# Ulixes-8/UNet-Implementations

Hardware: AMD Instinct MI355X
Metric: images/sec (512x512, bs/GPU=8) Our_UNet train step (higher is better)
Workload: dtype f32; 1 GPU; Our_UNet 6-stage 3-class 512x512 bs=8/GPU fp32 train step (fwd + Dice/wCE loss + bwd + SGD-Nesterov), train mode, HIP conv/IN/upsample kernels; global_batch=8, parallelism=dp1, world=1

## Files before the change

include/unet_hip.h:

```cpp
#ifndef UNET_HIP_H_
#define UNET_HIP_H_

#include <stddef.h>
#include <stdint.h>

#ifdef __cplusplus
extern "C" {
#endif

#define UNET_ABI_VERSION 11

#define UNET_OK 0
#define UNET_E_INVALID (-1)
#define UNET_E_LAUNCH (-2)
#define UNET_E_WORKSPACE (-3)

typedef void* unet_stream_t;

const char* unet_last_error(void);
int unet_abi_version(void);
int unet_device_count(void);

int unet_debug_set_chunk_limit(int64_t bytes);

// ... 235 lines not shown
                                const uint16_t* dy, float* dw_oihw, void* workspace,
                                size_t workspace_bytes, int N, int H, int W, int Cout,
                                unet_stream_t stream);

size_t unet_stem_in_bwd_weight_fold_workspace_bytes(int N, int H, int W, int Cout);
int unet_stem_in_bwd_weight_fold(const float* x, const uint8_t* image_hwc, const float* mean3,
                                 const float* std3, const float* g, const float* y,
                                 const float* mean, const float* rstd, const float* gamma,
                                 const float* beta, const float* mask, float slope,
                                 const void* partial, int tiles, float* dw_oihw, float* dgamma,
                                 float* dbeta, float* dbias, void* workspace,
                                 size_t workspace_bytes, int N, int H, int W, int Cout,
                                 unet_stream_t stream);

int unet_conv_in_bwd_weight_fold32_supported(int N, int H, int W, int Cx, int Cout);
size_t unet_conv_in_bwd_weight_fold32_workspace_bytes(int N, int H, int W);
int unet_conv_in_bwd_weight_fold32(const unet_act_src* x, float slope_x, float* g, const float* y,
                                   const float* mean, const float* rstd, const float* gamma,
                                   const float* beta, const float* mask, float slope,
                                   const void* partial, int tiles, float* dw_oihw, int ci_offset,
                                   int Cin_total, float* dgamma, float* dbeta, float* dbias,
                                   void* workspace, size_t workspace_bytes, int N, int H, int W,
                                   unet_stream_t stream);

int unet_conv_in_bwd_weight(const unet_act_src* x, float slope, const float* dy, float* dw_oihw,
                            int ci_offset, int Cin_total, int ksize, int stride, void* workspace,
                            size_t workspace_bytes, int N, int H, int W, int Cout,
                            unet_stream_t stream);
int unet_conv_in_bwd_weight_bf16x3(const unet_act_src* x, float slope, const float* dy, float* dw_oihw,
                            int ci_offset, int Cin_total, int ksize, int stride, void* workspace,
                            size_t workspace_bytes, int N, int H, int W, int Cout,
                            unet_stream_t stream);

int unet_upsample2x_in_fwd(const unet_act_src* x, float slope, float* up, int N, int h, int w,
                           unet_stream_t stream);

int unet_upsample2x_bwd_taps(const float* dy, float* D, int N, int h, int w, int C,
                             unet_stream_t stream);
int unet_resize_bilinear_fwd(const float* x, float* y, int planes, int h, int w, int H, int W,
                             unet_stream_t stream);
int unet_resize_bilinear_bwd(const float* gy, float* gx, int planes, int h, int w, int H, int W,
                             unet_stream_t stream);
size_t unet_conv3x3_up_bwd_weight_workspace_bytes(int N, int h, int w, int Cx, int Cout);
int unet_conv3x3_up_bwd_weight(const unet_act_src* x, float slope, const float* D, float* dw_oihw,
                               int ci_offset, int Cin_total, void* workspace,
                               size_t workspace_bytes, int N, int h, int w, int Cout,
// ... 220 lines not shown
```

unet-implementations_amd/_lib.py:

```python
import ctypes
import os
import subprocess

_HERE = os.path.dirname(os.path.abspath(__file__))
LIB_PATH = os.environ.get("UNET_HIP_LIB") or os.path.join(_HERE, "libunet_hip.so")
CSRC = os.path.join(_HERE, "csrc")

ABI_VERSION = 11

_c = ctypes
_p = _c.c_void_p
_i = _c.c_int
_f = _c.c_float
_sz = _c.c_size_t
_i64 = _c.c_int64



class ActSrc(ctypes.Structure):
    _fields_ = [("x", _p), ("C", _i), ("alpha", _p), ("beta", _p)]


_ps = _c.POINTER(ActSrc)

# ... 130 lines not shown
                                     _i, _p]),
    "unet_conv3x3_up_bwd_data_b16": (_i, [_p, _p, _i, _i, _p, _i, _i, _i, _i, _i, _i, _p]),
    "unet_conv3x3_up_bwd_data_bs_b16": (_i, [_p, _p, _i, _i, _p, _i, _i, _i, _i, _i, _i, _pbs, _p]),
    "unet_conv3x3_up_bwd_data_bs_b16_wb": (_i, [_p, _p, _p, _i, _i, _p, _i, _i, _i, _i, _i, _i, _pbs,
                                           _p]),
    "unet_head1x1_in_fwd_b16": (_i, [_ps, _f, _p, _p, _p, _i, _i, _i, _p]),
    "unet_head1x1_in_bwd_b16": (_i, [_ps, _f, _p, _p, _p, _p, _p, _p, _sz, _i, _i, _i, _p]),
    "unet_upsample2x_bwd_taps": (_i, [_p, _p, _i, _i, _i, _i, _p]),
    "unet_conv3x3_up_bwd_weight_workspace_bytes": (_sz, [_i, _i, _i, _i, _i]),
    "unet_conv3x3_up_bwd_weight": (_i, [_ps, _f, _p, _p, _i, _i, _p, _sz, _i, _i, _i, _i, _p]),
    "unet_conv3x3_up_bwd_data": (_i, [_p, _p, _i, _i, _p, _i, _i, _i, _i, _i, _i, _p]),
    "unet_head1x1_in_fwd": (_i, [_ps, _f, _p, _p, _p, _i, _i, _i, _p]),
    "unet_head1x1_in_bwd": (_i, [_ps, _f, _p, _p, _p, _p, _p, _p, _sz, _i, _i, _i, _p]),
    "unet_head1x1_in_bwd_bs": (_i, [_ps, _f, _p, _p, _p, _p, _p, _p, _sz, _i, _i, _i, _pbs, _p]),
    "unet_head1x1_in_bwd_bs_b16": (_i, [_ps, _f, _p, _p, _p, _p, _p, _p, _sz, _i, _i, _i, _pbs, _p]),
    "unet_stem_in_bwd_weight_fold_workspace_bytes": (_sz, [_i, _i, _i, _i]),
    "unet_stem_in_bwd_weight_fold": (_i, [_p, _p, _c.POINTER(_f), _c.POINTER(_f), _p, _p, _p, _p, _p,
                                          _p, _p, _f, _p, _i, _p, _p, _p, _p, _p, _sz, _i, _i, _i,
                                          _i, _p]),
    "unet_conv_in_bwd_weight_fold32_supported": (_i, [_i, _i, _i, _i, _i]),
    "unet_conv_in_bwd_weight_fold32_workspace_bytes": (_sz, [_i, _i, _i]),
    "unet_conv_in_bwd_weight_fold32": (_i, [_ps, _f, _p, _p, _p, _p, _p, _p, _p, _f, _p, _i, _p, _i,
                                            _i, _p, _p, _p, _p, _sz, _i, _i, _i, _p]),
    "unet_instnorm_bwd_merge_partials": (_i, [_p, _i, _p, _p, _i, _i, _i, _p]),
    "unet_head1x1_in_bwd_fold_workspace_bytes": (_sz, [_i, _i, _i]),
    "unet_head1x1_in_bwd_fold": (_i, [_ps, _f, _p, _p, _p, _p, _p, _p, _p, _p, _p, _sz, _i, _i, _i,
                                      _pbs, _p]),
    "unet_recon3x3_fwd": (_i, [_ps, _i, _f, _p, _p, _p, _i, _i, _i, _i, _p]),
    "unet_recon3x3_bwd_workspace_bytes": (_sz, [_i, _i, _i]),
    "unet_recon3x3_bwd": (_i, [_ps, _i, _f, _p, _p, _p, _p, _p, _p, _p, _sz, _i, _i, _i, _i, _pbs,
                               _p]),
    "unet_mse_loss_workspace_bytes": (_sz, [_i, _i, _i, _i]),
    "unet_mse_loss_fwd": (_i, [_p, _p, _i, _p, _p, _p, _sz, _i, _i, _i, _i, _p]),
    "unet_mse_loss_grad": (_i, [_p, _p, _i, _p, _p, _i, _i, _i, _i, _p]),
    "unet_adam_step": (_i, [_p, _p, _p, _p, _i64, _p, _i, _p]),
    "unet_ssim_workspace_bytes": (_sz, [_i, _i, _i, _i]),
    "unet_ssim_fwd": (_i, [_p, _p, _i, _c.POINTER(_f), _f, _f, _p, _p, _p, _c.c_double,
                           _c.c_double, _p, _sz, _i, _i, _i, _i, _p]),
    "unet_ssim_grad": (_i, [_p, _p, _i, _c.POINTER(_f), _f, _f, _p, _i, _c.c_double, _c.c_double,
                            _p, _i, _i, _i, _i, _p]),
    "unet_perceptual_prep": (_i, [_p, _p, _i, _c.POINTER(_f), _c.POINTER(_f), _p, _i, _i, _i, _p]),
    "unet_relu_maxpool2x2_fwd": (_i, [_p, _p, _i, _i, _i, _i, _p]),
    "unet_feature_mse_workspace_bytes": (_sz, [_i, _i, _i, _i]),
    "unet_feature_mse_fwd": (_i, [_p, _p, _p, _sz, _i, _i, _i, _i, _p]),
    "unet_perceptual_relu_bwd": (_i, [_p, _p, _f, _p, _p, _p, _i, _i, _i, _i, _p]),
    "unet_perceptual_stem_bwd_data": (_i, [_p, _p, _c.POINTER(_f), _p, _i, _i, _i, _i, _p]),
# ... 54 lines not shown
```

unet-implementations_amd/csrc/conv_wgrad.hip:

```cpp
#include "conv_params.h"
#include <vector>
#include "lds_asm.h"
#include <type_traits>
#include <utility>

namespace {
using unet_conv::act4;
using unet_conv::act4f;
template <int I> using template_ic = std::integral_constant<int, I>;
template <int B, int... I, typename F>
__device__ __forceinline__ void for_range_impl(std::integer_sequence<int, I...>, F&& f) {
  (f(template_ic<B + I>{}), ...);
}
template <int B, int E, typename F>
__device__ __forceinline__ void for_range(F&& f) {
  for_range_impl<B>(std::make_integer_sequence<int, (E > B ? E - B : 0)>{}, f);
}

struct WgradParams {
  const float* x;
  const float* dy;
  float* partial;
  int Cx, Cout;
  int N, H, W, Ho, Wo;
// ... 1500 lines not shown
  static_assert(lds <= 160 * 1024, "stages exceed the CU's LDS");
  return with_bool(p.alpha != nullptr, [&](auto act) {
    return launch_kernel<
        conv_wgrad_kernel<CI_T, CO_T, S, STRIDE, decltype(act)::value, float, float, 8>>(
        "conv_wgrad(8 waves)", wgrad_grid(p), 512, lds, stream, p);
  });
}

template <int CI_T, int CO_T, int STRIDE>
int launch_wgrad8_s(const WgradParams& p, int S, hipStream_t stream) {
  constexpr int NSB = (CI_T / 32) * (CO_T / 32);
  constexpr int SMAX = NSB == 1 ? (STRIDE == 1 ? 128 : 32) : NSB == 2 ? 64 : (STRIDE == 1 ? 64 : 32);
  if constexpr (SMAX >= 128) if (S == 128) return launch_wgrad8<CI_T, CO_T, 128, STRIDE>(p, stream);
  if constexpr (SMAX >= 64) if (S == 64) return launch_wgrad8<CI_T, CO_T, 64, STRIDE>(p, stream);
  if (S == 32) return launch_wgrad8<CI_T, CO_T, 32, STRIDE>(p, stream);
  if (S == 16) return launch_wgrad8<CI_T, CO_T, 16, STRIDE>(p, stream);
  unet_set_error("conv_wgrad(8 waves): no instantiation for S=%d", S);
  return UNET_E_INVALID;
}

constexpr int WW_XP = 4 * 18, WW_DP = 2 * 16;
constexpr int WW_BUF = 16 * 512;
constexpr size_t WW_LDS = (size_t)(4 * WW_BUF + (WW_XP + WW_DP) * 64) * sizeof(float);

template <bool ACT>
__global__ __launch_bounds__(512, 2) void conv_wgrad_wino_kernel(const WgradParams p) {
  extern __shared__ __attribute__((aligned(16))) float smem[];
  float* Vs = smem;
  float* Es = smem + 2 * WW_BUF;
  float* Rx = smem + 4 * WW_BUF;
  float* Rd = Rx + WW_XP * 64;

  const int tid = threadIdx.x, lane = tid & 63, wave = tid >> 6;
  int bid = blockIdx.x;
  const int co_t = bid % p.co_tiles; bid /= p.co_tiles;
  const int ci_t = bid % p.ci_tiles; bid /= p.ci_tiles;
  const int sp = bid;
  const int ci0 = ci_t * 64, co0 = co_t * 64;
  const int g_begin = sp * p.segs_per_block;
  const int g_end = min(g_begin + p.segs_per_block, p.total_segs);
  const int cw = p.W >> 4, th = p.H >> 1;

  const int xshift = (p.W + 1) * p.Cx;
  const __amdgpu_buffer_rsrc_t rsx = __builtin_amdgcn_make_buffer_rsrc(
      const_cast<float*>(p.x) - xshift, 0, (int)(p.x_bytes + 4u * (unsigned)xshift), 0x00020000);
  const __amdgpu_buffer_rsrc_t rsd = __builtin_amdgcn_make_buffer_rsrc(
      const_cast<float*>(p.dy), 0, (int)p.dy_bytes, 0x00020000);

  const int grp4 = (tid & 15) * 4;
  unsigned voffx[3], fx[3];
  float* xdst[3];
#pragma unroll
  for (int i = 0; i < 3; ++i) {
    const int pix = (tid + 512 * i) >> 4;
    const int prow = pix / 18, pcol = pix - prow * 18;
    voffx[i] = (unsigned)((prow * p.W + pcol) * p.Cx + ci0 + grp4) * 4u;
    fx[i] = (prow == 0 ? 1u : 0u) | (prow == 3 ? 2u : 0u) | (pcol == 0 ? 4u : 0u) |
            (pcol == 17 ? 8u : 0u) | (pix >= WW_XP ? 16u : 0u);
    xdst[i] = Rx + (pix < WW_XP ? pix : 0) * 64 + grp4;
  }
  const bool slot2 = tid + 1024 < WW_XP * 16;
  const int d_pixl = tid >> 4;
  const unsigned voffd = (unsigned)(((d_pixl >> 4) * p.W + (d_pixl & 15)) * p.Cout + co0 + grp4) * 4u;
  float* const ddst = Rd + d_pixl * 64 + grp4;
  f32x4 rx[3], rd;
  float okf[3] = {1.f, 1.f, 1.f};
  f32x4 ca = {1.f, 1.f, 1.f, 1.f}, cb = {0.f, 0.f, 0.f, 0.f};
  int l_cc, l_tr, l_n, l_g = g_begin;
  {
    const int r = g_begin / cw;
    l_cc = g_begin - r * cw;
    l_n = r / th;
    l_tr = r - l_n * th;
  }
  auto load_raw = [&]() {
    const unsigned m = (l_tr == 0 ? 1u : 0u) | (l_tr == th - 1 ? 2u : 0u) | (l_cc == 0 ? 4u : 0u) |
                       (l_cc == cw - 1 ? 8u : 0u) | 16u;
    const int pixbase = (l_n * p.H + 2 * l_tr) * p.W + 16 * l_cc;
#pragma unroll
    for (int i = 0; i < 3; ++i) {
      const bool ok = (fx[i] & m) == 0u;
      okf[i] = ok ? 1.f : 0.f;
      rx[i] = __builtin_bit_cast(f32x4, __builtin_amdgcn_raw_buffer_load_b128(
                                            rsx, ok ? voffx[i] : 0x80000000u, pixbase * p.Cx * 4, 0));
    }
    rd = __builtin_bit_cast(f32x4, __builtin_amdgcn_raw_buffer_load_b128(rsd, voffd,
                                                                          pixbase * p.Cout * 4, 0));
    if (ACT) {
      const size_t o = (size_t)l_n * p.Cx + ci0;
      ca = *reinterpret_cast<const f32x4*>(p.alpha + o + grp4);
      cb = *reinterpret_cast<const f32x4*>(p.beta + o + grp4);
    }
    if (l_g + 1 < g_end) {
      ++l_g;
      if (++l_cc == cw) { l_cc = 0; if (++l_tr == th) { l_tr = 0; ++l_n; } }
    }
  };
  auto store_x = [&](auto ic) {
    constexpr int i = decltype(ic)::value;
    f32x4 v = rx[i];
    if (ACT) v = act4f(v, ca, cb, p.slope, okf[i]);
    if (i < 2 || slot2) *reinterpret_cast<f32x4*>(xdst[i]) = v;
  };
  auto store_d = [&]() { *reinterpret_cast<f32x4*>(ddst) = rd; };

  const int t_pair = wave & 3;
  const int t_half = __builtin_amdgcn_readfirstlane(wave >> 2);
  const unsigned t_xa = lds_addr(Rx + (4 * t_pair) * 64 + lane);
  const unsigned t_da = lds_addr(Rd + (4 * t_pair) * 64 + lane);
  const int t_off = t_pair * 128 + ((lane * 2) ^ (32 * (t_pair & 1)));
  float* const t_vdst = Vs + t_off;
  float* const t_edst = Es + t_off;
  f32x2v tq[6];
  auto tv_rd = [&](auto ac) {
    constexpr int a = decltype(ac)::value;
    constexpr int r0 = a == 0 ? 0 : (a == 1 ? 1 : (a == 2 ? 2 : 3));
    constexpr int r1 = a == 0 ? 2 : (a == 1 ? 2 : 1);
    tq[0] = lds_rd2st64<r0 * 18 + 0, r1 * 18 + 0>(t_xa);
    tq[1] = lds_rd2st64<r0 * 18 + 1, r1 * 18 + 1>(t_xa);
    tq[2] = lds_rd2st64<r0 * 18 + 2, r1 * 18 + 2>(t_xa);
    tq[3] = lds_rd2st64<r0 * 18 + 3, r1 * 18 + 3>(t_xa);
    tq[4] = lds_rd2st64<r0 * 18 + 4, r1 * 18 + 4>(t_xa);
    tq[5] = lds_rd2st64<r0 * 18 + 5, r1 * 18 + 5>(t_xa);
  };
  auto tv_wr = [&](auto ac, auto bc) {
    constexpr int a = decltype(ac)::value;
    constexpr int B = decltype(bc)::value;
// ... 86 lines not shown
      constexpr int NR = T ? n_reads(T ? x - 8 : 0, HF) : 0;
      if constexpr (x == 8) {
        asm volatile("s_waitcnt lgkmcnt(0)" ::: "memory");
        __builtin_amdgcn_s_barrier();
        asm volatile("" ::: "memory");
      }
      if constexpr (T) t_reads(template_ic<(T ? x - 8 : 0)>{}, hc);
      if constexpr (x + 1 < 16) frag(bc, template_ic<x + 1>{});
      lds_wait<(x + 1 < 16 ? 3 : 0) + NR>(fa[x & 1], fb0[x & 1], fb1[x & 1]);
      __builtin_amdgcn_sched_barrier(0);
      mm(xc);
      if constexpr (T) {
        lds_wait6<3>(tq[0], tq[1], tq[2], tq[3], tq[4], tq[5]);
        t_writes(template_ic<(T ? x - 8 : 0)>{}, hc, NB{});
      }
      if constexpr (x < 3) store_x(template_ic<(x < 3 ? x : 0)>{});
      if constexpr (x == 3) store_d();
      if constexpr (x == 4) load_raw();
      __builtin_amdgcn_sched_barrier(0);
    });
  };
  auto k_loop = [&](auto hc) {
    load_raw();
    for_range<0, 3>(store_x);
    store_d();
    load_raw();
    __syncthreads();
    for_range<0, 4>([&](auto kc) {
      t_reads(kc, hc);
      lds_wait6<0>(tq[0], tq[1], tq[2], tq[3], tq[4], tq[5]);
      t_writes(kc, hc, template_ic<0>{});
    });
    for (int g = g_begin; g < g_end; g += 2) {
      chunk_body(template_ic<0>{}, hc);
      if (g + 1 < g_end) chunk_body(template_ic<1>{}, hc);
    }
  };
  if (g_begin < g_end) {
    if (t_half == 0) k_loop(template_ic<0>{}); else k_loop(template_ic<1>{});
  }

#pragma unroll
  for (int x = 0; x < 16; ++x) {
    const float sc = (((x >> 2) == 1 || (x >> 2) == 2) ? 0.5f : 1.f) * (((x & 3) == 1 || (x & 3) == 2) ? 0.5f : 1.f);
    if (sc != 1.f) {
#pragma unroll
      for (int b = 0; b < 2; ++b) acc[x][b] *= sc;
    }
  }
#pragma unroll
  for (int b = 0; b < 2; ++b)
#pragma unroll
    for (int r = 0; r < 4; ++r) {
      float s[3][4];
#pragma unroll
      for (int j = 0; j < 4; ++j) {
        s[0][j] = acc[0 + j][b][r] + acc[4 + j][b][r] + acc[8 + j][b][r];
        s[1][j] = acc[4 + j][b][r] - acc[8 + j][b][r];
        s[2][j] = acc[4 + j][b][r] + acc[8 + j][b][r] + acc[12 + j][b][r];
      }
// ... 316 lines not shown
    return false;
  return c32 == 2 || (long long)N * (H / 8) * (W / 32) >= 256;
}
WgradPlan make_plan_wino32(int N, int H, int W) {
  WgradPlan pl{};
  const long long t = (long long)N * (H / 8) * (W / 32);
  pl.nw = 8; pl.ci_t = pl.co_t = 32; pl.npp = 1; pl.S = 16;
  pl.split = (int)(t < 256 ? t : 256);
  pl.total_segs = (int)t; pl.segs_per_block = 1; pl.segs_per_row = W / 32;
  pl.ws_floats = slab_ws_floats(pl.split, (size_t)9 * 32 * 32);
  return pl;
}
int launch_wgrad_wino32(const WgradParams& p, hipStream_t stream) {
  const int ntiles = p.N * (p.H / 8) * (p.W / 32);
  return with_bool(p.alpha != nullptr, [&](auto act) {
    return launch_kernel<conv_wgrad_wino32_kernel<decltype(act)::value>>(
        "conv_wgrad_wino32", dim3((unsigned)(ntiles < 256 ? ntiles : 256)), 512, WQ_LDS, stream, p,
        ntiles);
  });
}

int launch_wgrad_wino(const WgradParams& p, hipStream_t stream) {
  return with_bool(p.alpha != nullptr, [&](auto act) {
    return launch_kernel<conv_wgrad_wino_kernel<decltype(act)::value>>(
        "conv_wgrad_wino", wgrad_grid(p), 512, WW_LDS, stream, p);
  });
}

bool wgrad_wino_ok(int N, int H, int W, int Cx, int Cout, int stride) {
  if (stride != 1 || Cx % 64 || Cout % 64 || H % 2 || W % 16) return false;
  const long long chunks = (long long)N * (H / 2) * (W / 16);
  return chunks >= 32 && chunks < (1LL << 30);
}

WgradPlan make_plan_wino(int N, int H, int W, int Cx, int Cout) {
  WgradPlan pl{};
  pl.nw = 8; pl.ci_t = pl.co_t = 64; pl.npp = 2; pl.S = 16;
  pl.segs_per_row = W / 16;
  pl.total_segs = N * (H / 2) * (W / 16);
  pl.segs_per_block = ceil_div(
      pl.total_segs, wgrad_split(256, (Cx / 64) * (Cout / 64), ceil_div(pl.total_segs, 8)));
  return with_slabs(pl, Cx, Cout);
}

template <int CI_T, int CO_T, int S, int STRIDE>
int launch_wgrad(const WgradParams& p, hipStream_t stream) {
  constexpr int PW = (S - 1) * STRIDE + 3;
  constexpr size_t stages = 2 * (size_t)(3 * PW * CI_T + S * CO_T) * sizeof(float);
// ... 158 lines not shown
  }
  if (pl.ci_t == 32 && pl.co_t == 64) {
    if (stride == 1)
      return pl.S == 32 ? launch_wgrad<32, 64, 32, 1>(p, stream)
                        : launch_wgrad<32, 64, 16, 1>(p, stream);
    return pl.S == 32 ? launch_wgrad<32, 64, 32, 2>(p, stream)
                      : launch_wgrad<32, 64, 16, 2>(p, stream);
  }
  if (stride == 1)
    return pl.S == 32 ? launch_wgrad<64, 64, 32, 1>(p, stream)
                      : launch_wgrad<64, 64, 16, 1>(p, stream);
  return launch_wgrad<64, 64, 16, 2>(p, stream);
}

enum WgradForm { WF_STEM, WF_WINO, WF_WINO32, WF_DIRECT, WF_TAPS };

struct WgradCall {
  const void* x = nullptr;
  const unsigned char* x_u8 = nullptr;
  const float* u8_mean_std = nullptr;
  const void* dy = nullptr;
  const StemNormW* stem_fold = nullptr;
  const StemNormW* fold32 = nullptr;
  const float* alpha = nullptr;
  const float* beta = nullptr;
  float slope = 0.f;
  bool b16 = false;
  int prec = 0;
  bool center_only = false;
  bool taps = false;
  float* dw = nullptr;
  int ci_offset = 0, Cin_total = 0;
  float* db = nullptr;
  void* workspace = nullptr;
  size_t workspace_bytes = 0;
  int N = 0, H = 0, W = 0, Cx = 0, Cout = 0, stride = 1;

  int Ho() const { return (H - 1) / stride + 1; }
  int Wo() const { return (W - 1) / stride + 1; }
  int dy_channels() const { return taps ? 9 * Cout : Cout; }
};

struct WgradSel {
  WgradForm form;
  PlanOpts opt;
  int nmax;
// ... 53 lines not shown
                        hipStream_t stream) {
  const long long es = c.b16 ? 2 : 4;
  const size_t E = (size_t)9 * c.Cx * c.Cout;
  const size_t x_img = (size_t)c.H * c.W * c.Cx * es;
  const size_t dy_img = (size_t)c.Ho() * c.Wo() * c.dy_channels() * es;
  *nslab = 0;
  for (int nb = 0; nb < c.N; nb += s.nmax) {
    const int nc = c.N - nb < s.nmax ? c.N - nb : s.nmax;
    const WgradPlan pl = wgrad_plan(c, s.form, s.opt, nc);
    WgradParams p{};
    p.x = reinterpret_cast<const float*>(static_cast<const char*>(c.x) + nb * x_img);
    p.dy = reinterpret_cast<const float*>(static_cast<const char*>(c.dy) + nb * dy_img);
    p.b16 = c.b16;
    p.partial = ws + (size_t)*nslab * E; p.Cx = c.Cx; p.Cout = c.Cout;
    p.N = nc; p.H = c.H; p.W = c.W; p.Ho = c.Ho(); p.Wo = c.Wo();
    p.segs_per_row = pl.segs_per_row; p.total_segs = pl.total_segs;
    p.segs_per_block = pl.segs_per_block; p.split = pl.split;
    p.ci_tiles = c.Cx / pl.ci_t; p.co_tiles = c.Cout / pl.co_t;
    p.x_bytes = (unsigned)(nc * x_img);
    p.dy_bytes = (unsigned)(nc * dy_img);
    p.alpha = c.alpha ? c.alpha + (size_t)nb * c.Cx : nullptr;
    p.beta = c.alpha ? c.beta + (size_t)nb * c.Cx : nullptr;
    p.slope = c.slope;
    if (c.fold32) {
      UNET_REQUIRE(s.form == WF_WINO32 && nc == c.N, "conv_in_bwd_weight_fold32: not a shape of "
                   "the 32-channel Winograd weight gradient");
      const StemNormW& f = *c.fold32;
      p.fy = f.y; p.fmu = f.mu; p.frstd = f.rstd; p.fgamma = f.gamma; p.fbeta = f.beta;
      p.fmask = f.mask; p.fcoef = f.coef; p.fsums = f.sums;
      p.fdgamma = f.dgamma; p.fdbeta = f.dbeta; p.fdbias = f.dbias; p.fslope = f.slope;
    }
    const int rc = s.form == WF_WINO32 ? launch_wgrad_wino32(p, stream)
                   : s.form == WF_WINO ? launch_wgrad_wino(p, stream)
                   : s.form == WF_TAPS ? launch_wgrad_taps_plan(p, pl, stream)
                                       : launch_wgrad_plan(p, pl, c.stride, c.prec, stream);
    if (rc != UNET_OK) return rc;
    *nslab += pl.split;
  }
  return UNET_OK;
}

int launch_wgrad_stem(const WgradCall& c, const WgradPlan& pl, float* ws, hipStream_t stream) {
  StemNormW nm{};
  if (c.stem_fold) {
    UNET_REQUIRE(c.W % SW_PIX == 0 && !c.b16, "stem_in_bwd_weight_fold: needs W %% %d == 0 and an "
                 "fp32 gradient", SW_PIX);
    nm = *c.stem_fold;
  }
  if (c.x_u8) {
    UNET_REQUIRE(c.W % SW_PIX == 0, "stem_u8_bwd_weight: needs W %% %d == 0", SW_PIX);
// ... 342 lines not shown
  const size_t coef_b = align_up((size_t)N * 32 * sizeof(float2), 256);
  if (workspace_bytes < 2 * coef_b) {
    unet_set_error("conv_in_bwd_weight_fold32: workspace too small");
    return UNET_E_WORKSPACE;
  }
  char* ws = reinterpret_cast<char*>(workspace);
  StemNormW f{};
  f.y = y; f.mu = mean; f.rstd = rstd; f.gamma = gamma; f.beta = beta; f.mask = mask;
  f.coef = reinterpret_cast<const float2*>(ws);
  f.sums = reinterpret_cast<const float2*>(ws + coef_b);
  f.dgamma = dgamma; f.dbeta = dbeta; f.dbias = dbias; f.slope = slope;
  const int rc = unet_instnorm_bwd_merge_partials(partial, tiles, ws, ws + coef_b, N, H * W, 32,
                                                  stream);
  if (rc != UNET_OK) return rc;
  WgradCall c;
  set_source(c, x, slope_x);
  c.dy = g; c.fold32 = &f;
  c.dw = dw_oihw; c.ci_offset = ci_offset; c.Cin_total = Cin_total;
  c.workspace = ws + 2 * coef_b; c.workspace_bytes = workspace_bytes - 2 * coef_b;
  c.N = N; c.H = H; c.W = W; c.Cout = 32;
  return conv_bwd_weight_impl(c, (hipStream_t)stream);
}

extern "C" size_t unet_conv3x3_up_bwd_weight_workspace_bytes(int N, int h, int w, int Cx, int Cout) {
  if (N <= 0 || h <= 0 || w <= 0 || Cx <= 0 || Cout <= 0) return 0;
  size_t m = 0;
  for (const bool b16 : {false, true}) {
    WgradCall c;
    c.taps = true; c.b16 = b16;
    c.N = N; c.H = h; c.W = w; c.Cx = Cx; c.Cout = Cout;
    const size_t f = wgrad_ws_floats(c, wgrad_select(c, 0));
    if (f > m) m = f;
  }
  return m * sizeof(float);
}

static int up_bwd_weight_impl(const WgradCall& c, hipStream_t stream) {
  UNET_REQUIRE(c.x && c.dy && c.dw && c.workspace, "conv3x3_up_bwd_weight: null pointer");
  UNET_REQUIRE(c.Cx > 0 && c.Cx % 32 == 0 && c.Cout > 0 && c.Cout % 32 == 0 && c.N > 0 && c.H > 0 &&
                   c.W > 0,
               "conv3x3_up_bwd_weight: bad shape Cx=%d Cout=%d", c.Cx, c.Cout);
  UNET_REQUIRE(c.ci_offset >= 0 && c.ci_offset + c.Cx <= c.Cin_total, "conv3x3_up_bwd_weight: bad ci slice");
  UNET_REQUIRE(!c.alpha || c.beta, "conv3x3_up_bwd_weight: alpha without beta");
  const WgradSel sel = wgrad_select(c, 0);
  UNET_REQUIRE(sel.nmax >= 1, "conv3x3_up_bwd_weight: one image exceeds the 2 GiB buffer-descriptor range");
  const size_t need = wgrad_ws_floats(c, sel) * sizeof(float);
// ... 54 lines not shown
```

unet-implementations_amd/ops.py:

```python
import ctypes
import functools
import struct
import threading

import torch

from ._lib import ActSrc, BwdStats, check, lib


_raw_stream = getattr(torch._C, "_cuda_getCurrentRawStream", None)
_raw_device = getattr(torch._C, "_cuda_getDevice", None)


def _stream():
    if _raw_stream is not None and _raw_device is not None:
        return _raw_stream(_raw_device())
    return torch.cuda.current_stream().cuda_stream


class KernelTimer:

    def __init__(self, only=None):
        self.only = only
        self.records = []
# ... 751 lines not shown
    if isinstance(x, U8Image) or xt.dtype != torch.float32 or g.dtype != torch.float32 or \
            xt.shape[:3] != g.shape[:3]:
        return False
    N, H, W, Cx = xt.shape
    return bool(lib().unet_conv_in_bwd_weight_fold32_supported(N, H, W, Cx, g.shape[3]))


def conv_in_bwd_weight_fold32(x, slope_x, g, y, mean, rstd, gamma, beta, mask, slope, partials,
                              dw_oihw, ci_offset, dgamma, dbeta, dbias):
    x, rx = _act(x)
    N, H, W, _ = x.shape
    assert dw_oihw.shape[0] == 32 and dw_oihw.is_contiguous() and g.is_contiguous()
    ws = _wgrad_ws(lib().unet_conv_in_bwd_weight_fold32_workspace_bytes(N, H, W), g)
    t0 = _begin("wgrad")
    check(lib().unet_conv_in_bwd_weight_fold32(
        rx, slope_x, _ptr(g), _ptr(y), _ptr(mean), _ptr(rstd), _ptr(gamma), _ptr(beta), _ptr(mask),
        slope, _ptr(partials[0]), partials[1], _ptr(dw_oihw), ci_offset, dw_oihw.shape[1],
        _ptr(dgamma), _ptr(dbeta), _ptr(dbias), _ptr(ws), ws.numel(), N, H, W, _stream()))
    if t0 is not None:
        _end_conv(t0, "conv_wgrad", 2.0 * N * H * W * 9 * 32 * 32, 3, True)
    return g


def upsample2x_in_fwd(x, slope):
    x, rx = _act(x)
    N, h, w, C = x.shape
    b16 = _is_b16(x.x)
    up = (_b16 if b16 else _f32)((N, 2 * h, 2 * w, C), x.x)
    t0 = _begin()
    check(_twin("unet_upsample2x_in_fwd", b16)(rx, slope, _ptr(up), N, h, w, _stream()))
    if t0 is not None:
        _timer.end("upsample2x_fwd", 0.0, 1, t0,
                   nbytes=x.x.element_size() * (x.x.numel() + up.numel()))
    return up


def upsample2x_bwd_taps(dy):
    N, H2, W2, C = dy.shape
    b16 = _is_b16(dy)
    D = (_b16 if b16 else _f32)((N, H2 // 2, W2 // 2, 9 * C), dy)
    t0 = _begin()
    check(_twin("unet_upsample2x_bwd_taps", b16)(_ptr(dy), _ptr(D), N, H2 // 2, W2 // 2, C,
                                                 _stream()))
    if t0 is not None:
        _timer.end("upsample2x_bwd_taps", 0.0, 1, t0,
                   nbytes=dy.element_size() * dy.numel() * (1 + 9 / 4))
# ... 622 lines not shown
```

unet-implementations_amd/unet.py:

```python
from typing import Dict, List, Optional, Tuple, Type, Union

import torch
import torch.nn as nn

from . import ops


class SpatialDropout2d(nn.Module):

    def __init__(self, drop_prob):
        super().__init__()
        self.drop_prob = drop_prob

    def extra_repr(self):
        return f"drop_prob={self.drop_prob}"

    def draw_mask(self, n, channels, device):
        mask = torch.empty(n, channels, 1, 1, device=device).bernoulli_(1 - self.drop_prob)
        return mask.div_(1 - self.drop_prob).view(n, channels)

    def forward(self, x):
        if not self.training or self.drop_prob == 0:
            return x
        return x * self.draw_mask(x.size(0), x.size(1), x.device).view(x.size(0), x.size(1), 1, 1)
# ... 258 lines not shown
        self._fusion_layer = None
        self._build_bottleneck(common)
        self.decoder_stages = nn.ModuleList()
        for s in range(n_stages - 1):
            lvl = n_stages - 2 - s
            self.decoder_stages.append(
                UpBlock(features_per_stage[lvl + 1], features_per_stage[lvl],
                        features_per_stage[lvl], kernel_sizes[lvl],
                        n_convs=n_conv_per_stage_decoder[lvl],
                        spatial_dropout_rate=decoder_dropout_rates[s], **common))
        self._build_head(features_per_stage[0], num_classes)
        self.initialize_weights()
        self._plan = None
        self._arena = None
        self._grad_arena = None
        self._offsets = None
        self.dropout_mask_override = None
        self.grad_ready_hook = None
        self.matmul_precision = "fp32"
        self.fused_pipeline = True
        self.winograd = True
        self.fullres_folds = True
        self.wgrad32_folds = True
        self.input_mean, self.input_std = ops.IMAGENET_MEAN, ops.IMAGENET_STD

    def _build_bottleneck(self, common):
        """Hook for variants that add modules between encoder and decoder (CLIPUNet)."""

    def _build_head(self, in_features, out_channels):
        self.segmentation_output = nn.Conv2d(in_features, out_channels, kernel_size=1, stride=1,
                                             padding=0, bias=True)

    def _head_module(self):
        return self.segmentation_output

    def _check_head(self):
        head = self.segmentation_output
        if _as_int(head.kernel_size) != 1 or head.in_channels != 32 or head.out_channels != 3:
            raise NotImplementedError("the HIP head kernel is the 32 -> 3 1x1 convolution")

    def _head_fwd(self, walk, cur):
        head = self.segmentation_output
        hw = head.weight.detach().view(head.out_channels, -1)
        if walk.fused:
            return ops.head1x1_in_fwd(cur, walk.slope, hw, head.bias.detach())
        return ops.head1x1_fwd(cur, hw, head.bias.detach())
# ... 352 lines not shown
        rec = self.saved[i]
        l, st, x0, x1, low = rec.layer, rec.st, rec.x0, rec.x1, rec.low
        fused, slope = self.fused, self.slope
        gv = (lambda p: None) if grad_only else self.model._grad_view
        need_dx = i > stop
        need_dx1 = rec.skip_dst is not None and rec.skip_dst > stop
        dbg = getattr(self.model, "_debug_capture", None)
        if dbg is not None:
            dbg.append((l.name, "ga", g_a.clone()))
        nn_, rec.nxt = rec.nxt, None
        nxt = self.saved[i - 1].next_norm() \
            if fused and need_dx and not (grad_only and i - 1 == stop) else None
        dw = gv(l.conv.weight)
        want_dw = l.conv.weight.requires_grad and not grad_only
        partials = (nn_.partial, nn_.tiles) if nn_ is not None and nn_.tiles > 0 else None
        if i == 0 and fused and want_dw and partials is not None and dbg is None and \
                self.mode == "fp32" and x1 is None and low is None and l.ksize == 3 and \
                self.model.fullres_folds and ops.stem_in_bwd_weight_fold_supported(x0, g_a):
            ops.stem_in_bwd_weight_fold(x0, g_a, rec.y, st[0], st[1], l.norm.weight.detach(),
                                        l.norm.bias.detach(), rec.mask, l.slope, partials, dw,
                                        gv(l.norm.weight), gv(l.norm.bias), gv(l.conv.bias))
            return None, None
        xw = x1 if low is not None else x0
        fold32 = fused and want_dw and partials is not None and dbg is None and \
            self.mode == "fp32" and not self.x3 and l.ksize == 3 and l.stride == 1 and \
            self.model.wgrad32_folds and not (nn_ is not None and nn_.applied) and \
            (low is not None or x1 is None) and xw is not None and \
            not _hooked(rec.bwd_hooks, "_backward_hooks") and \
            ops.conv_in_bwd_weight_fold32_supported(xw, g_a)
        if nn_ is not None and nn_.applied:
            dy = g_a
        elif fold32:
            dy = ops.conv_in_bwd_weight_fold32(
                xw, slope, g_a, rec.y, st[0], st[1], l.norm.weight.detach(), l.norm.bias.detach(),
                rec.mask, l.slope, partials, dw, low.shape[3] if low is not None else 0,
                gv(l.norm.weight), gv(l.norm.bias), gv(l.conv.bias))
        else:
            dy = ops.instnorm_lrelu_drop_bwd(g_a, rec.y, st[0], st[1], l.norm.weight.detach(),
                                             l.norm.bias.detach(), rec.mask, l.slope,
                                             gv(l.norm.weight), gv(l.norm.bias), gv(l.conv.bias),
                                             partials=partials)
        if dbg is not None:
            dbg.append((l.name, "dy", dy.clone()))
        if low is not None:
            C0 = low.shape[3]
            D = ops.upsample2x_bwd_taps(dy) if (want_dw or need_dx) else None
            if want_dw:
                ops.conv3x3_up_bwd_weight(low, slope, D, dw, 0)
                if not fold32:
                    ops.conv_in_bwd_weight(x1, slope, dy, dw, C0, 3, 1, x3=self.x3)
            g_low = ops.conv3x3_up_bwd_data(D, rec.wd, 0, C0, nxt=nxt,
                                            wd3=rec.wd3 if ops._is_b16(D) else None) \
                if need_dx else None
            dx1 = ops.conv3x3_bwd_data(dy, rec.wd, C0, x1.shape[3], x1.shape[1], x1.shape[2], 1,
                                       wd3=rec.wd3,
                                       bf16="bf16x3" if rec.wd3 is not None else False,
                                       ud=rec.ud1) if need_dx1 else None
            return g_low, dx1
        if want_dw and fused and fold32:
            want_dw = False
        elif want_dw and fused:
            ops.conv_in_bwd_weight(x0, slope, dy, dw, 0, l.ksize, l.stride, x3=self.x3)
            if x1 is not None:
                ops.conv_in_bwd_weight(x1, slope, dy, dw, x0.shape[3], l.ksize, l.stride,
                                       x3=self.x3)
            want_dw = False
        if l.ksize == 1:
            if want_dw:
                dw2d = dw.view(dw.shape[0], dw.shape[1])
                ops.conv1x1_bwd_weight(x0, dy, dw2d, 0)
                if x1 is not None:
                    ops.conv1x1_bwd_weight(x1, dy, dw2d, x0.shape[3])
            dx0 = ops.conv1x1_bwd_data(dy, rec.wd, 0, x0.shape[3]) if need_dx else None
            return dx0, None
        if want_dw:
            ops.conv3x3_bwd_weight(x0, dy, dw, 0, l.stride, bf16=self.mode)
            if x1 is not None:
                ops.conv3x3_bwd_weight(x1, dy, dw, x0.shape[3], l.stride, bf16=self.mode)
        dx0 = dx1 = None
        N, H, W, C0 = x0.shape
        if need_dx:
            dx0 = ops.conv3x3_bwd_data(dy, rec.wd, 0, C0, H, W, l.stride, out=dx0_acc,
# ... 182 lines not shown
```

Measured before the change: 475.8 images/s.

## Fold InstanceNorm/LReLU backward into 64-channel Winograd weight-gradient kernel

Extends the existing fold that computes the InstanceNorm+LeakyReLU+dropout backward inside the weight-gradient kernel from the 32-channel Winograd path to the 64-input-channel Winograd path. The kernel now loads per-(n,channel) norm parameters into extra LDS rows, computes dz from y and g on the fly, writes dz back to global memory, and block 0 computes the norm parameter gradients. This removes a separate instnorm backward pass over the activation gradient, at the cost of more LDS per block, an extra barrier in the k-loop, and extra loads of y.

```diff
diff --git a/include/unet_hip.h b/include/unet_hip.h
--- a/include/unet_hip.h
+++ b/include/unet_hip.h
@@ -281,6 +281,16 @@
                                    int Cin_total, float* dgamma, float* dbeta, float* dbias,
                                    void* workspace, size_t workspace_bytes, int N, int H, int W,
                                    unet_stream_t stream);
+
+int unet_conv_in_bwd_weight_fold_supported(int N, int H, int W, int Cx, int Cout);
+size_t unet_conv_in_bwd_weight_fold_workspace_bytes(int N, int H, int W, int Cx, int Cout);
+int unet_conv_in_bwd_weight_fold(const unet_act_src* x, float slope_x, float* g, const float* y,
+                                 const float* mean, const float* rstd, const float* gamma,
+                                 const float* beta, const float* mask, float slope,
+                                 const void* partial, int tiles, float* dw_oihw, int ci_offset,
+                                 int Cin_total, float* dgamma, float* dbeta, float* dbias,
+                                 void* workspace, size_t workspace_bytes, int N, int H, int W,
+                                 int Cout, unet_stream_t stream);
 
 int unet_conv_in_bwd_weight(const unet_act_src* x, float slope, const float* dy, float* dw_oihw,
                             int ci_offset, int Cin_total, int ksize, int stride, void* workspace,
diff --git a/unet-implementations_amd/_lib.py b/unet-implementations_amd/_lib.py
--- a/unet-implementations_amd/_lib.py
+++ b/unet-implementations_amd/_lib.py
@@ -176,6 +176,10 @@
     "unet_conv_in_bwd_weight_fold32_workspace_bytes": (_sz, [_i, _i, _i]),
     "unet_conv_in_bwd_weight_fold32": (_i, [_ps, _f, _p, _p, _p, _p, _p, _p, _p, _f, _p, _i, _p, _i,
                                             _i, _p, _p, _p, _p, _sz, _i, _i, _i, _p]),
+    "unet_conv_in_bwd_weight_fold_supported": (_i, [_i, _i, _i, _i, _i]),
+    "unet_conv_in_bwd_weight_fold_workspace_bytes": (_sz, [_i, _i, _i, _i, _i]),
+    "unet_conv_in_bwd_weight_fold": (_i, [_ps, _f, _p, _p, _p, _p, _p, _p, _p, _f, _p, _i, _p, _i,
+                                          _i, _p, _p, _p, _p, _sz, _i, _i, _i, _i, _p]),
     "unet_instnorm_bwd_merge_partials": (_i, [_p, _i, _p, _p, _i, _i, _i, _p]),
     "unet_head1x1_in_bwd_fold_workspace_bytes": (_sz, [_i, _i, _i]),
     "unet_head1x1_in_bwd_fold": (_i, [_ps, _f, _p, _p, _p, _p, _p, _p, _p, _p, _p, _sz, _i, _i, _i,
diff --git a/unet-implementations_amd/csrc/conv_wgrad.hip b/unet-implementations_amd/csrc/conv_wgrad.hip
--- a/unet-implementations_amd/csrc/conv_wgrad.hip
+++ b/unet-implementations_amd/csrc/conv_wgrad.hip
@@ -1546,6 +1546,9 @@
 constexpr int WW_XP = 4 * 18, WW_DP = 2 * 16;
 constexpr int WW_BUF = 16 * 512;
 constexpr size_t WW_LDS = (size_t)(4 * WW_BUF + (WW_XP + WW_DP) * 64) * sizeof(float);
+constexpr int WW_FROWS = 7 * 64;
+constexpr size_t WW_LDS_FOLD = WW_LDS + (size_t)2 * WW_FROWS * sizeof(float);
+static_assert(WW_LDS_FOLD <= 160 * 1024, "the fold's rows live in the LDS the stages leave");
 
 template <bool ACT>
 __global__ __launch_bounds__(512, 2) void conv_wgrad_wino_kernel(const WgradParams p) {
@@ -1554,6 +1557,7 @@
   float* Es = smem + 2 * WW_BUF;
   float* Rx = smem + 4 * WW_BUF;
   float* Rd = Rx + WW_XP * 64;
+  float* Fc = Rd + WW_DP * 64;
 
   const int tid = threadIdx.x, lane = tid & 63, wave = tid >> 6;
   int bid = blockIdx.x;
@@ -1570,6 +1574,9 @@
       const_cast<float*>(p.x) - xshift, 0, (int)(p.x_bytes + 4u * (unsigned)xshift), 0x00020000);
   const __amdgpu_buffer_rsrc_t rsd = __builtin_amdgcn_make_buffer_rsrc(
       const_cast<float*>(p.dy), 0, (int)p.dy_bytes, 0x00020000);
+  const bool fold = p.fy != nullptr;
+  const __amdgpu_buffer_rsrc_t rsy = __builtin_amdgcn_make_buffer_rsrc(
+      const_cast<float*>(p.fy), 0, fold ? (int)p.dy_bytes : 0, 0x00020000);
 
   const int grp4 = (tid & 15) * 4;
   unsigned voffx[3], fx[3];
@@ -1597,10 +1604,35 @@
     l_n = r / th;
     l_tr = r - l_n * th;
   }
+  f32x4 ry = {0.f, 0.f, 0.f, 0.f};
+  int d_n = 0, d_off = 0, f_n = -1, f_left = g_end - g_begin;
+  auto ldg = [](const float* q) { return *(const __attribute__((address_space(1))) float*)q; };
+  auto load_rows = [&](int n) {
+    if (tid < 64) {
+      const int c = co0 + tid;
+      const size_t o = (size_t)n * p.Cout + c;
+      float* const r = Fc + (n & 1) * WW_FROWS + tid;
+      const float mu = ldg(p.fmu + o), rs = ldg(p.frstd + o);
+      const float al = ldg(p.fgamma + c) * rs;
+      r[0] = mu;
+      r[64] = rs;
+      r[128] = al;
+      r[192] = __builtin_fmaf(-mu, al, ldg(p.fbeta + c));
+      r[256] = p.fmask ? ldg(p.fmask + o) : 1.f;
+      r[320] = ldg(&p.fcoef[o].x);
+      r[384] = ldg(&p.fcoef[o].y);
+    }
+  };
   auto load_raw = [&]() {
     const unsigned m = (l_tr == 0 ? 1u : 0u) | (l_tr == th - 1 ? 2u : 0u) | (l_cc == 0 ? 4u : 0u) |
                        (l_cc == cw - 1 ? 8u : 0u) | 16u;
     const int pixbase = (l_n * p.H + 2 * l_tr) * p.W + 16 * l_cc;
+    if (fold) {
+      if (l_n != f_n) { load_rows(l_n); f_n = l_n; }
+      d_n = l_n;
+      d_off = pixbase * p.Cout;
+      ry = __builtin_bit_cast(f32x4, __builtin_amdgcn_raw_buffer_load_b128(rsy, voffd, d_off * 4, 0));
+    }
 #pragma unroll
     for (int i = 0; i < 3; ++i) {
       const bool ok = (fx[i] & m) == 0u;
@@ -1626,7 +1658,16 @@
     if (ACT) v = act4f(v, ca, cb, p.slope, okf[i]);
     if (i < 2 || slot2) *reinterpret_cast<f32x4*>(xdst[i]) = v;
   };
-  auto store_d = [&]() { *reinterpret_cast<f32x4*>(ddst) = rd; };
+  auto store_d = [&]() {
+    if (fold && f_left > 0) {
+      --f_left;
+      const f32x4* const fr = reinterpret_cast<const f32x4*>(Fc + (d_n & 1) * WW_FROWS + grp4);
+      rd = in_bwd_dz4(rd, ry, fr[0], fr[16], fr[32], fr[48], fr[64], p.fslope, fr[80], fr[96]);
+      *(__attribute__((address_space(1))) f32x4*)(
+          reinterpret_cast<char*>(const_cast<float*>(p.dy) + d_off) + voffd) = rd;
+    }
+    *reinterpret_cast<f32x4*>(ddst) = rd;
+  };
 
   const int t_pair = wave & 3;
   const int t_half = __builtin_amdgcn_readfirstlane(wave >> 2);
@@ -1759,6 +1800,7 @@
   };
   auto k_loop = [&](auto hc) {
     load_raw();
+    if (fold) __syncthreads();
     for_range<0, 3>(store_x);
     store_d();
     load_raw();
@@ -1773,6 +1815,9 @@
       if (g + 1 < g_end) chunk_body(template_ic<1>{}, hc);
     }
   };
+  if (fold && blockIdx.x == 0)
+    in_bwd_param_grads(p.fsums, p.fcoef, p.fgamma, p.frstd, p.N, p.H * p.W, p.Cout, tid, 512,
+                       p.fdgamma, p.fdbeta, p.fdbias);
   if (g_begin < g_end) {
     if (t_half == 0) k_loop(template_ic<0>{}); else k_loop(template_ic<1>{});
   }
@@ -2135,8 +2180,11 @@
 
 int launch_wgrad_wino(const WgradParams& p, hipStream_t stream) {
   return with_bool(p.alpha != nullptr, [&](auto act) {
-    return launch_kernel<conv_wgrad_wino_kernel<decltype(act)::value>>(
-        "conv_wgrad_wino", wgrad_grid(p), 512, WW_LDS, stream, p);
+    constexpr auto kern = conv_wgrad_wino_kernel<decltype(act)::value>;
+    UNET_SET_DYN_LDS(kern, WW_LDS_FOLD);
+    hipLaunchKernelGGL(kern, wgrad_grid(p), dim3(512), p.fy ? WW_LDS_FOLD : WW_LDS, stream, p);
+    UNET_CHECK_LAUNCH("conv_wgrad_wino");
+    return UNET_OK;
   });
 }
 
@@ -2341,6 +2389,7 @@
   const void* dy = nullptr;
   const StemNormW* stem_fold = nullptr;
   const StemNormW* fold32 = nullptr;
+  const StemNormW* fold_wino = nullptr;
   const float* alpha = nullptr;
   const float* beta = nullptr;
   float slope = 0.f;
@@ -2440,10 +2489,13 @@
     p.alpha = c.alpha ? c.alpha + (size_t)nb * c.Cx : nullptr;
     p.beta = c.alpha ? c.beta + (size_t)nb * c.Cx : nullptr;
     p.slope = c.slope;
-    if (c.fold32) {
-      UNET_REQUIRE(s.form == WF_WINO32 && nc == c.N, "conv_in_bwd_weight_fold32: not a shape of "
-                   "the 32-channel Winograd weight gradient");
-      const StemNormW& f = *c.fold32;
+    if (c.fold32 || c.fold_wino) {
+      UNET_REQUIRE(!c.fold32 || (s.form == WF_WINO32 && nc == c.N), "conv_in_bwd_weight_fold32: "
+                   "not a shape of the 32-channel Winograd weight gradient");
+      UNET_REQUIRE(!c.fold_wino || (s.form == WF_WINO && nc == c.N && c.Cx == 64),
+                   "conv_in_bwd_weight_fold: not a 64-input-channel shape of the Winograd weight "
+                   "gradient");
+      const StemNormW& f = c.fold32 ? *c.fold32 : *c.fold_wino;
       p.fy = f.y; p.fmu = f.mu; p.frstd = f.rstd; p.fgamma = f.gamma; p.fbeta = f.beta;
       p.fmask = f.mask; p.fcoef = f.coef; p.fsums = f.sums;
       p.fdgamma = f.dgamma; p.fdbeta = f.dbeta; p.fdbias = f.dbias; p.fslope = f.slope;
@@ -2832,6 +2884,61 @@
   return conv_bwd_weight_impl(c, (hipStream_t)stream);
 }
 
+extern "C" int unet_conv_in_bwd_weight_fold_supported(int N, int H, int W, int Cx, int Cout) {
+  if (N <= 0 || H <= 0 || W <= 0 || Cx != 64 || Cout <= 0) return 0;
+  WgradCall c;
+  c.N = N; c.H = H; c.W = W; c.Cx = Cx; c.Cout = Cout;
+  const WgradSel s = wgrad_select(c, unet_conv::c32_winograd_flag());
+  return s.form == WF_WINO && s.nmax >= N ? 1 : 0;
+}
+
+extern "C" size_t unet_conv_in_bwd_weight_fold_workspace_bytes(int N, int H, int W, int Cx,
+                                                               int Cout) {
+  if (N <= 0 || H <= 0 || W <= 0 || Cx <= 0 || Cout <= 0) return 0;
+  return 2 * align_up((size_t)N * Cout * sizeof(float2), 256) +
+         unet_conv3x3_bwd_weight_workspace_bytes(N, H, W, Cx, Cout, 1);
+}
+
+extern "C" int unet_conv_in_bwd_weight_fold(const unet_act_src* x, float slope_x, float* g,
+                                            const float* y, const float* mean, const float* rstd,
+                                            const float* gamma, const float* beta,
+                                            const float* mask, float slope, const void* partial,
+                                            int tiles, float* dw_oihw, int ci_offset,
+                                            int Cin_total, float* dgamma, float* dbeta,
+                                            float* dbias, void* workspace, size_t workspace_bytes,
+                                            int N, int H, int W, int Cout, unet_stream_t stream) {
+  const int rc0 = check_conv_in("conv_in_bwd_weight_fold", x, 3, 1);
+  if (rc0 != UNET_OK) return rc0;
+  UNET_REQUIRE(g && y && mean && rstd && gamma && beta && partial && tiles > 0 && workspace,
+               "conv_in_bwd_weight_fold: null pointer");
+  UNET_REQUIRE(unet_conv_in_bwd_weight_fold_supported(N, H, W, x->C, Cout),
+               "conv_in_bwd_weight_fold: N=%d H=%d W=%d Cx=%d Cout=%d is not a 64-input-channel "
+               "shape of the Winograd weight gradient", N, H, W, x->C, Cout);
+  UNET_REQUIRE(x->x != g && x->x != y, "conv_in_bwd_weight_fold: g is rewritten in place and "
+               "cannot be the layer's operand");
+  const size_t coef_b = align_up((size_t)N * Cout * sizeof(float2), 256);
+  if (workspace_bytes < 2 * coef_b) {
+    unet_set_error("conv_in_bwd_weight_fold: workspace too small");
+    return UNET_E_WORKSPACE;
+  }
+  char* ws = reinterpret_cast<char*>(workspace);
+  StemNormW f{};
+  f.y = y; f.mu = mean; f.rstd = rstd; f.gamma = gamma; f.beta = beta; f.mask = mask;
+  f.coef = reinterpret_cast<const float2*>(ws);
+  f.sums = reinterpret_cast<const float2*>(ws + coef_b);
+  f.dgamma = dgamma; f.dbeta = dbeta; f.dbias = dbias; f.slope = slope;
+  const int rc = unet_instnorm_bwd_merge_partials(partial, tiles, ws, ws + coef_b, N, H * W, Cout,
+                                                  stream);
+  if (rc != UNET_OK) return rc;
+  WgradCall c;
+  set_source(c, x, slope_x);
+  c.dy = g; c.fold_wino = &f;
+  c.dw = dw_oihw; c.ci_offset = ci_offset; c.Cin_total = Cin_total;
+  c.workspace = ws + 2 * coef_b; c.workspace_bytes = workspace_bytes - 2 * coef_b;
+  c.N = N; c.H = H; c.W = W; c.Cout = Cout;
+  return conv_bwd_weight_impl(c, (hipStream_t)stream);
+}
+
 extern "C" size_t unet_conv3x3_up_bwd_weight_workspace_bytes(int N, int h, int w, int Cx, int Cout) {
   if (N <= 0 || h <= 0 || w <= 0 || Cx <= 0 || Cout <= 0) return 0;
   size_t m = 0;
diff --git a/unet-implementations_amd/ops.py b/unet-implementations_amd/ops.py
--- a/unet-implementations_amd/ops.py
+++ b/unet-implementations_amd/ops.py
@@ -797,6 +797,32 @@
     return g
 
 
+def conv_in_bwd_weight_fold_supported(x, g):
+    xt = x.x if isinstance(x, Act) else x
+    if isinstance(x, U8Image) or xt.dtype != torch.float32 or g.dtype != torch.float32 or \
+            xt.shape[:3] != g.shape[:3]:
+        return False
+    N, H, W, Cx = xt.shape
+    return bool(lib().unet_conv_in_bwd_weight_fold_supported(N, H, W, Cx, g.shape[3]))
+
+
+def conv_in_bwd_weight_fold(x, slope_x, g, y, mean, rstd, gamma, beta, mask, slope, partials,
+                            dw_oihw, ci_offset, dgamma, dbeta, dbias):
+    x, rx = _act(x)
+    N, H, W, Cx = x.shape
+    Cout = g.shape[3]
+    assert dw_oihw.shape[0] == Cout and dw_oihw.is_contiguous() and g.is_contiguous()
+    ws = _wgrad_ws(lib().unet_conv_in_bwd_weight_fold_workspace_bytes(N, H, W, Cx, Cout), g)
+    t0 = _begin("wgrad")
+    check(lib().unet_conv_in_bwd_weight_fold(
+        rx, slope_x, _ptr(g), _ptr(y), _ptr(mean), _ptr(rstd), _ptr(gamma), _ptr(beta), _ptr(mask),
+        slope, _ptr(partials[0]), partials[1], _ptr(dw_oihw), ci_offset, dw_oihw.shape[1],
+        _ptr(dgamma), _ptr(dbeta), _ptr(dbias), _ptr(ws), ws.numel(), N, H, W, Cout, _stream()))
+    if t0 is not None:
+        _end_conv(t0, "conv_wgrad", 2.0 * N * H * W * 9 * Cx * Cout, 3, True)
+    return g
+
+
 def upsample2x_in_fwd(x, slope):
     x, rx = _act(x)
     N, h, w, C = x.shape
diff --git a/unet-implementations_amd/unet.py b/unet-implementations_amd/unet.py
--- a/unet-implementations_amd/unet.py
+++ b/unet-implementations_amd/unet.py
@@ -304,6 +304,7 @@
         self.winograd = True
         self.fullres_folds = True
         self.wgrad32_folds = True
+        self.wgrad_wino_folds = True
         self.input_mean, self.input_std = ops.IMAGENET_MEAN, ops.IMAGENET_STD
 
     def _build_bottleneck(self, common):
@@ -702,16 +703,21 @@
                                         gv(l.norm.weight), gv(l.norm.bias), gv(l.conv.bias))
             return None, None
         xw = x1 if low is not None else x0
-        fold32 = fused and want_dw and partials is not None and dbg is None and \
-            self.mode == "fp32" and not self.x3 and l.ksize == 3 and l.stride == 1 and \
-            self.model.wgrad32_folds and not (nn_ is not None and nn_.applied) and \
-            (low is not None or x1 is None) and xw is not None and \
-            not _hooked(rec.bwd_hooks, "_backward_hooks") and \
-            ops.conv_in_bwd_weight_fold32_supported(xw, g_a)
+        fold_op = None
+        if fused and want_dw and partials is not None and dbg is None and \
+                self.mode == "fp32" and not self.x3 and l.ksize == 3 and l.stride == 1 and \
+                not (nn_ is not None and nn_.applied) and \
+                (low is not None or x1 is None) and xw is not None and \
+                not _hooked(rec.bwd_hooks, "_backward_hooks"):
+            if self.model.wgrad32_folds and ops.conv_in_bwd_weight_fold32_supported(xw, g_a):
+                fold_op = ops.conv_in_bwd_weight_fold32
+            elif self.model.wgrad_wino_folds and ops.conv_in_bwd_weight_fold_supported(xw, g_a):
+                fold_op = ops.conv_in_bwd_weight_fold
+        folded = fold_op is not None
         if nn_ is not None and nn_.applied:
             dy = g_a
-        elif fold32:
-            dy = ops.conv_in_bwd_weight_fold32(
+        elif folded:
+            dy = fold_op(
                 xw, slope, g_a, rec.y, st[0], st[1], l.norm.weight.detach(), l.norm.bias.detach(),
                 rec.mask, l.slope, partials, dw, low.shape[3] if low is not None else 0,
                 gv(l.norm.weight), gv(l.norm.bias), gv(l.conv.bias))
@@ -727,7 +733,7 @@
             D = ops.upsample2x_bwd_taps(dy) if (want_dw or need_dx) else None
             if want_dw:
                 ops.conv3x3_up_bwd_weight(low, slope, D, dw, 0)
-                if not fold32:
+                if not folded:
                     ops.conv_in_bwd_weight(x1, slope, dy, dw, C0, 3, 1, x3=self.x3)
             g_low = ops.conv3x3_up_bwd_data(D, rec.wd, 0, C0, nxt=nxt,
                                             wd3=rec.wd3 if ops._is_b16(D) else None) \
@@ -737,7 +743,7 @@
                                        bf16="bf16x3" if rec.wd3 is not None else False,
                                        ud=rec.ud1) if need_dx1 else None
             return g_low, dx1
-        if want_dw and fused and fold32:
+        if want_dw and fused and folded:
             want_dw = False
         elif want_dw and fused:
             ops.conv_in_bwd_weight(x0, slope, dy, dw, 0, l.ksize, l.stride, x3=self.x3)
```

New measurement: 476.6 images/s, median of 5. No clear change (+0.2%).
